# quentinll/pertrenderer

Measured on AMD Instinct MI355X. Metric: rendered frames/sec + ms/backward, 256² img, 50 faces/px, 8 samples, higher is better.
Workload: dtype f32; 1 GPU; cfg2 pose-opt step: sphere_642 (1280 faces), 256x256, faces_per_pixel=50, Sr=Sa=8 Gaussian, sigma=1e-3 gamma=1e-2, blur=ln(1e4-1)*sigma, fwd + L2 loss (native) + bwd + Adam step on the pose (lr 5e-2); image_size=256, faces_per_pixel=50, nb_samples=8, rast_samples=8, batch=1, execution=graph, parallelism=single GPU

## Files before the change

### pertrenderer_amd/csrc/pr_rast.hip

```cpp
#include <cstdlib>
#include <type_traits>

#include <hip/hip_fp16.h>

#include "pr_common.h"

namespace pr {
namespace {

constexpr float kEps = 1e-8f;
constexpr int kTile = 4;

struct V2 {
  float x, y;
};

template <bool FAST = false>
PR_DEV float dv(float a, float b) {
  if constexpr (FAST) return a * __builtin_amdgcn_rcpf(b);
  else return a / b;
}

PR_DEV float edge_fn(V2 p, V2 a, V2 b) { return (p.x - a.x) * (b.y - a.y) - (p.y - a.y) * (b.x - a.x); }

// ... 42 lines not shown

PR_DEV float ndc(int i, int S1, int S2) {
  float range = 2.0f;
  if (S1 > S2) range = ((float)S1 * range) / (float)S2;
  const float off = range / 2.0f;
  return -off + (range * (float)i + off) / (float)S1;
}

struct FaceRec {
  float4 a;
  float4 b;
  float4 c;
  float4 d;
  float4 e;
  float4 f;
};

PR_DEV uint32_t half_bits(__half h) { return (uint32_t)__half_as_ushort(h); }
PR_DEV uint2 pack_box(float xmin, float xmax, float ymin, float ymax) {
  return make_uint2(half_bits(__float2half_rd(xmin)) | (half_bits(__float2half_ru(xmax)) << 16),
                    half_bits(__float2half_rd(ymin)) | (half_bits(__float2half_ru(ymax)) << 16));
}
PR_DEV float4 unpack_box(uint2 b) {
  return make_float4(__half2float(__ushort_as_half((unsigned short)(b.x & 0xffffu))),
                     __half2float(__ushort_as_half((unsigned short)(b.x >> 16))),
                     __half2float(__ushort_as_half((unsigned short)(b.y & 0xffffu))),
                     __half2float(__ushort_as_half((unsigned short)(b.y >> 16))));
}

PR_DEV void write_face_rec(const float v[9], float blur, int cull_backfaces, FaceRec* out, uint2* bbox) {
  const float x0 = v[0], y0 = v[1], z0 = v[2], x1 = v[3], y1 = v[4], z1 = v[5], x2 = v[6], y2 = v[7], z2 = v[8];
  const float r = sqrtf(blur);
  float xmin = fminf(x0, fminf(x1, x2)) - r, xmax = fmaxf(x0, fmaxf(x1, x2)) + r;
  float ymin = fminf(y0, fminf(y1, y2)) - r, ymax = fmaxf(y0, fmaxf(y1, y2)) + r;
  const float zmax = fmaxf(z0, fmaxf(z1, z2));
  const float area = edge_fn(V2{x0, y0}, V2{x1, y1}, V2{x2, y2});
  const bool back = area < 0.f;
  const bool zero_area = area <= kEps && area >= -kEps;
  const bool valid = !(zmax < 0.f || (cull_backfaces && back) || zero_area);
  if (!valid) { xmin = ymin = __builtin_inff(); xmax = ymax = -__builtin_inff(); }
  const float d01x = x1 - x0, d01y = y1 - y0, d12x = x2 - x1, d12y = y2 - y1, d20x = x0 - x2, d20y = y0 - y2;
  FaceRec rec;
  rec.a = make_float4(x0, y0, z0, x1);
  rec.b = make_float4(y1, z1, x2, y2);
  rec.c = make_float4(z2, xmin, xmax, ymin);
  rec.d = make_float4(ymax, edge_fn(V2{x2, y2}, V2{x0, y0}, V2{x1, y1}) + kEps, d01x * d01x + d01y * d01y,
                      d12x * d12x + d12y * d12y);
  rec.e = make_float4(d01x, d01y, d12x, d12y);
  rec.f = make_float4(d20x, d20y, d20x * d20x + d20y * d20y, fminf(z0, fminf(z1, z2)));
  *out = rec;
  *bbox = pack_box(xmin, xmax, ymin, ymax);
}

struct BinGrid {
  int bs, nx, ny, cap;
  int* count;
  int* list;
  int H, W;
};

PR_DEV void bin_rect(const BinGrid& g, int bx, int by, float& xmin, float& xmax, float& ymin, float& ymax) {
  const int c0 = bx * g.bs, c1 = min(c0 + g.bs - 1, g.W - 1), r0 = by * g.bs, r1 = min(r0 + g.bs - 1, g.H - 1);
  xmax = ndc(g.W - 1 - c0, g.W, g.H); xmin = ndc(g.W - 1 - c1, g.W, g.H);
  ymax = ndc(g.H - 1 - r0, g.H, g.W); ymin = ndc(g.H - 1 - r1, g.H, g.W);
}

PR_DEV void pix_range(float vmin, float vmax, int S1, int S2, int& lo, int& hi) {
  float range = 2.0f;
  if (S1 > S2) range = ((float)S1 * range) / (float)S2;
  const float off = range / 2.0f;
  const float ilo = fminf(fmaxf(((vmin + off) * (float)S1 - off) / range, -2.f), (float)S1 + 1.f);
  const float ihi = fminf(fmaxf(((vmax + off) * (float)S1 - off) / range, -2.f), (float)S1 + 1.f);
  lo = max(0, (int)floorf((float)(S1 - 1) - ihi) - 1);
  hi = min(S1 - 1, (int)ceilf((float)(S1 - 1) - ilo) + 1);
}

PR_DEV void bin_face(const BinGrid& g, int n, int64_t f, uint2 packed) {
  const float4 bb = unpack_box(packed);
  if (!(bb.x <= bb.y && bb.z <= bb.w)) return;
  int c0, c1, r0, r1;
  pix_range(bb.x, bb.y, g.W, g.H, c0, c1);
  pix_range(bb.z, bb.w, g.H, g.W, r0, r1);
  if (c0 > c1 || r0 > r1) return;
  const int bx0 = c0 / g.bs, nbx = c1 / g.bs - bx0 + 1, by0 = r0 / g.bs, nby = r1 / g.bs - by0 + 1;
  auto hits = [&](int bx, int by) {
    float xmin, xmax, ymin, ymax;
    bin_rect(g, bx, by, xmin, xmax, ymin, ymax);
    return !(bb.x > xmax || bb.y < xmin || bb.z > ymax || bb.w < ymin);
  };
  if (nbx * nby <= 16) {
    int b[16], c[16];
#pragma unroll
    for (int k = 0; k < 16; ++k) {
      const int bx = bx0 + k % nbx, by = by0 + k / nbx;
      b[k] = k < nbx * nby && hits(bx, by) ? (n * g.ny + by) * g.nx + bx : -1;
    }
#pragma unroll
    for (int k = 0; k < 16; ++k) c[k] = b[k] >= 0 ? atomicAdd(g.count + b[k], 1) : g.cap;
#pragma unroll
    for (int k = 0; k < 16; ++k)
      if (c[k] < g.cap) g.list[(int64_t)b[k] * g.cap + c[k]] = (int)f;
    return;
  }
  for (int by = by0; by < by0 + nby; ++by) {
    for (int bx = bx0; bx < bx0 + nbx; ++bx) {
      if (!hits(bx, by)) continue;
      const int bi = (n * g.ny + by) * g.nx + bx;
      const int c = atomicAdd(g.count + bi, 1);
      if (c < g.cap) g.list[(int64_t)bi * g.cap + c] = (int)f;
    }
  }
}

PR_DEV int mesh_of_sorted(const int64_t* first, int N, int64_t f) {
  int lo = 0, hi = N - 1;
  while (lo < hi) {
    const int mid = (lo + hi + 1) >> 1;
    if (first[mid] <= f) lo = mid;
    else hi = mid - 1;
  }
  return lo;
}

__global__ void face_prep_kernel(const float* fv, int64_t F, float blur_v, const float* blur_dev, int cull_backfaces,
                                 FaceRec* out, uint2* bbox, BinGrid bins, const int64_t* mesh_first, int N) {
  const float blur = blur_dev ? *blur_dev : blur_v;
  for (int64_t f = (int64_t)blockIdx.x * blockDim.x + threadIdx.x; f < F; f += (int64_t)gridDim.x * blockDim.x) {
    float v[9];
#pragma unroll
    for (int i = 0; i < 9; ++i) v[i] = fv[f * 9 + i];
    write_face_rec(v, blur, cull_backfaces, out + f, bbox + f);
    if (bins.count) bin_face(bins, mesh_of_sorted(mesh_first, N, f), f, bbox[f]);
  }
}

PR_DEV int divmod_small(int i, int d, float inv_d, int& r) {
  int q = (int)((float)i * inv_d);
  r = i - q * d;
  if (r < 0) { --q; r += d; }
  else if (r >= d) { ++q; r -= d; }
  return q;
}

PR_DEV bool key_less(float za, int fa, float zb, int fb) { return za < zb || (za == zb && fa < fb); }

PR_DEV float seg_dist2_d(V2 p, V2 a, float bax, float bay, float l2, V2 b) {
  const float bx = p.x - b.x, by = p.y - b.y;
  const float db = bx * bx + by * by;
  float t = (bax * (p.x - a.x) + bay * (p.y - a.y)) / l2;
  t = t < 0.f ? 0.f : (t > 1.f ? 1.f : t);
  const float qx = a.x + t * bax, qy = a.y + t * bay;
  const float dx = p.x - qx, dy = p.y - qy;
  const float ds = dx * dx + dy * dy;
  return l2 <= kEps ? db : ds;
}

template <bool PERSP, bool CLIP>
PR_DEV void face_eval(const FaceRec& r, V2 p, float bc[3], float& pz, bool& inside, float& d) {
  const V2 v0{r.a.x, r.a.y}, v1{r.a.w, r.b.x}, v2{r.b.z, r.b.w};
  const float z0 = r.a.z, z1 = r.b.y, z2 = r.c.x;
  const float area = r.d.y;
  const float e0 = (p.x - v1.x) * r.e.w - (p.y - v1.y) * r.e.z;
  const float e1 = (p.x - v2.x) * r.f.y - (p.y - v2.y) * r.f.x;
  const float e2 = (p.x - v0.x) * r.e.y - (p.y - v0.y) * r.e.x;
  float b[3] = {e0 / area, e1 / area, e2 / area};
  if constexpr (PERSP) {
    const float t0 = b[0] * z1 * z2, t1 = z0 * b[1] * z2, t2 = z0 * z1 * b[2];
    float s = t0 + t1 + t2;
    s = s > kEps ? s : kEps;
    b[0] = t0 / s; b[1] = t1 / s; b[2] = t2 / s;
  }
  if constexpr (CLIP) {
    clip_fwd(b, bc);
  } else {
    bc[0] = b[0]; bc[1] = b[1]; bc[2] = b[2];
  }
  pz = bc[0] * z0 + bc[1] * z1 + bc[2] * z2;
  inside = b[0] > 0.f && b[1] > 0.f && b[2] > 0.f;
  const float d01 = seg_dist2_d(p, v0, r.e.x, r.e.y, r.d.z, v1);
  const float d02 = seg_dist2_d(p, v0, -r.f.x, -r.f.y, r.f.z, v2);
  const float d12 = seg_dist2_d(p, v1, r.e.z, r.e.w, r.d.w, v2);
  d = d01 < d02 ? d01 : d02;
  d = d < d12 ? d : d12;
}

// ... 60 lines not shown
  pz = bc[0] * z0 + bc[1] * z1 + bc[2] * z2;
  const bool inside = b[0] > 0.f && b[1] > 0.f && b[2] > 0.f;
  bool near = dfast < blur - margin;
  if (!inside && !near && !(dfast > blur + margin)) {
    const float d01 = seg_dist2_d(p, v0, r.e.x, r.e.y, r.d.z, v1);
    const float d02 = seg_dist2_d(p, v0, -r.f.x, -r.f.y, r.f.z, v2);
    const float d12 = seg_dist2_d(p, v1, r.e.z, r.e.w, r.d.w, v2);
    float d = d01 < d02 ? d01 : d02;
    d = d < d12 ? d : d12;
    near = d < blur;
  }
  return !(pz < 0.f) && (inside || near);
}

PR_DEV bool in_bbox(const FaceRec& r, V2 p) {
  return !(p.x < r.c.y || p.x > r.c.z || p.y < r.c.w || p.y > r.d.x);
}

#ifdef PR_RAST_PROFILE
constexpr unsigned kProfTiles = 1 << 16;
__device__ long long g_rast_prof[kProfTiles * 16];
#define PR_STAMP(i) (stamp[i] += (long long)__builtin_amdgcn_s_memtime() - t_, t_ = __builtin_amdgcn_s_memtime())
#else
#define PR_STAMP(i) ((void)0)
#endif

template <int SL> struct RastCfg {
  static constexpr int CAP = SL == 1 ? 512 : (SL == 2 ? 256 : 128);
#ifndef PR_RAST_G4
#define PR_RAST_G4 2
#endif
  static constexpr int G = SL == 1 ? 4 : (SL >= 4 ? PR_RAST_G4 : 2);
#ifndef PR_RAST_CH4
#define PR_RAST_CH4 16
#endif
  static constexpr int CH = SL >= 4 ? PR_RAST_CH4 : 64;
  static_assert(CAP <= 8 * 64, "suffix-min pass holds CAP / 64 <= 8 entries per lane");
};
#ifndef PR_RAST_QPAD
template <int SL> constexpr int rast_qpad() { return SL == 4 ? 1 : 0; }
#else
template <int SL> constexpr int rast_qpad() { return PR_RAST_QPAD; }
#endif
#ifndef PR_RAST_MERGE
#define PR_RAST_MERGE 1
#endif
#ifndef PR_RAST_FRAGC
#define PR_RAST_FRAGC 1
#endif
#ifndef PR_RAST_CULLU
#define PR_RAST_CULLU 16
#endif
constexpr int kCullU = PR_RAST_CULLU;

template <int NT>
PR_DEV void bitonic_sort(float* key, int* val, int n2, int tid) {
  for (int k = 2; k <= n2; k <<= 1) {
    for (int j = k >> 1; j > 0; j >>= 1) {
      for (int i = tid; i < n2; i += NT) {
        const int ixj = i ^ j;
        if (ixj > i) {
          const bool up = (i & k) == 0;
          const float a = key[i], b = key[ixj];
          if ((a > b) == up) {
            key[i] = b; key[ixj] = a;
            const int t = val[i]; val[i] = val[ixj]; val[ixj] = t;
          }
        }
      }
      __syncthreads();
    }
  }
}

template <int E>
PR_DEV void wave_bitonic_sort(float (&key)[E], int (&val)[E], int lane) {
#pragma unroll
  for (int k = 2; k <= E * 64; k <<= 1) {
#pragma unroll
    for (int j = k >> 1; j > 0; j >>= 1) {
      if (j >= 64) {
        const int je = j >> 6;
#pragma unroll
        for (int e = 0; e < E; ++e) {
          const int pe = e ^ je;
          if (pe > e) {
            const bool up = ((e * 64 + lane) & k) == 0;
            const float a = key[e], b = key[pe];
            if ((a > b) == up) {
              key[e] = b; key[pe] = a;
              const int t = val[e]; val[e] = val[pe]; val[pe] = t;
            }
          }
        }
      } else {
#pragma unroll
        for (int e = 0; e < E; ++e) {
          const float ok = __shfl_xor(key[e], j);
          const int ov = __shfl_xor(val[e], j);
          const int i = e * 64 + lane;
          const bool up = (i & k) == 0, lower = (lane & j) == 0;
          const bool take = lower == up ? (ok < key[e]) : (ok > key[e]);
          if (take) { key[e] = ok; val[e] = ov; }
        }
      }
    }
// ... 17 lines not shown
PR_HD size_t rast_fwd_wave_bytes(int K) {
  using C = RastCfg<SL>;
  const size_t b = C::CH * sizeof(FaceRec) + (size_t)K * (64 / SL + rast_qpad<SL>()) * 8 + 64 * 4 + C::CH * 12;
  return (b + 15) / 16 * 16;
}

template <int SL>
size_t rast_fwd_lds_sl(int K, int NW) {
  return NW * rast_fwd_wave_bytes<SL>(K) + (size_t)RastCfg<SL>::CAP * 12 + 16;
}

size_t rast_fwd_lds(int K, int SL, int NW = 1) {
  return SL == 8 ? rast_fwd_lds_sl<8>(K, 1)
                 : SL == 4 ? rast_fwd_lds_sl<4>(K, NW) : (SL == 2 ? rast_fwd_lds_sl<2>(K, 1) : rast_fwd_lds_sl<1>(K, 1));
}

template <int SL>
PR_DEV int from_slice(int v, int s) {
  if constexpr (SL == 1) {
    return v;
  } else if constexpr (SL == 2) {
    switch (s) {
      case 0: return __builtin_amdgcn_update_dpp(0, v, 0xA0, 0xf, 0xf, false);
      default: return __builtin_amdgcn_update_dpp(0, v, 0xF5, 0xf, 0xf, false);
    }
  } else if constexpr (SL == 8) {
    return __shfl(v, (int)(__lane_id() & ~7u) | s);
  } else {
    switch (s) {
      case 0: return __builtin_amdgcn_update_dpp(0, v, 0x00, 0xf, 0xf, false);
      case 1: return __builtin_amdgcn_update_dpp(0, v, 0x55, 0xf, 0xf, false);
      case 2: return __builtin_amdgcn_update_dpp(0, v, 0xAA, 0xf, 0xf, false);
      default: return __builtin_amdgcn_update_dpp(0, v, 0xFF, 0xf, 0xf, false);
    }
  }
}

template <int SL>
PR_DEV int quad_rot(int v, int r) {
  if constexpr (SL == 2) {
    return __builtin_amdgcn_update_dpp(0, v, 0xB1, 0xf, 0xf, false);
  } else if constexpr (SL == 8) {
    const unsigned l = __lane_id();
    return __shfl(v, (int)((l & ~7u) | ((l + (unsigned)r) & 7u)));
  } else {
    switch (r) {
      case 1: return __builtin_amdgcn_update_dpp(0, v, 0x39, 0xf, 0xf, false);
      case 2: return __builtin_amdgcn_update_dpp(0, v, 0x4E, 0xf, 0xf, false);
      default: return __builtin_amdgcn_update_dpp(0, v, 0x93, 0xf, 0xf, false);
    }
  }
}

PR_DEV void ring_tile(int b, int m, int& tx, int& ty) {
  int r = (int)(__builtin_sqrtf((float)b) * 0.5f);
  while (4 * (r + 1) * (r + 1) <= b) ++r;
  while (4 * r * r > b) --r;
  const int k = b - 4 * r * r, s = 2 * r + 2, c0 = m / 2 - r - 1;
  if (k < s) { tx = c0 + k; ty = c0; }
  else if (k < 2 * s - 2) { tx = c0 + s - 1; ty = c0 + 1 + (k - s); }
  else if (k < 3 * s - 2) { tx = c0 + s - 1 - (k - (2 * s - 2)); ty = c0 + s - 1; }
  else { tx = c0; ty = c0 + s - 2 - (k - (3 * s - 2)); }
}

#ifndef PR_RAST_WPE
#define PR_RAST_WPE 1
#endif
#ifndef PR_RAST_DUO_WPE
#define PR_RAST_DUO_WPE 1
#endif
template <int SL, bool PERSP, bool CLIP, bool FRAG, int NW>
__global__ void __launch_bounds__(64 * NW, NW == 2 ? PR_RAST_DUO_WPE : PR_RAST_WPE)
    rast_fwd_kernel(PRRastArgs a, const FaceRec* __restrict__ faces, const uint2* __restrict__ fbox, int ring,
                    BinGrid bins) {
  constexpr int TW = SL >= 4 ? 4 : 8, TH = 64 / SL / TW, TP = TW * TH;
  constexpr int kCap = RastCfg<SL>::CAP, kGroup = RastCfg<SL>::G, CH = RastCfg<SL>::CH;
  constexpr int QS = TP + rast_qpad<SL>();
  constexpr int NT = 64 * NW;
  extern __shared__ float smem[];
  const int K = a.K;
  const int tid = threadIdx.x, lane = tid & 63, wv = NW == 2 ? tid >> 6 : 0;
  const int pix = lane / SL, slice = lane % SL;
  const size_t wbytes = rast_fwd_wave_bytes<SL>(K);
  char* wbase = reinterpret_cast<char*>(smem) + wv * wbytes;
  FaceRec* lrec = reinterpret_cast<FaceRec*>(wbase);
  float2* q = reinterpret_cast<float2*>(lrec + CH);
  int* qsz = reinterpret_cast<int*>(q + (size_t)K * QS);
  int* lcf = qsz + 64;
  float* lcs = reinterpret_cast<float*>(lcf + CH);
  float* lmg = lcs + CH;
  int* lfid = reinterpret_cast<int*>(reinterpret_cast<char*>(smem) + NW * wbytes);
  float* lkey = reinterpret_cast<float*>(lfid + kCap);
  float* lsuf = lkey;
  int* lidx = reinterpret_cast<int*>(lkey + kCap);
  int64_t* lctl = reinterpret_cast<int64_t*>(lidx + kCap);
  const int n = blockIdx.z;
  const int H = a.H, W = a.W;
  int tile_x = blockIdx.x, tile_y = blockIdx.y;
  if (ring & 1) {
    const int b = blockIdx.y * gridDim.x + blockIdx.x;
    if (gridDim.y == gridDim.x) {
      ring_tile(b, gridDim.x, tile_x, tile_y);
    } else {
      ring_tile(b >> 1, gridDim.x, tile_x, tile_y);
      tile_y = 2 * tile_y + (b & 1);
    }
  }
  const int row0 = tile_y * TH, col0 = tile_x * TW;
  const int row = row0 + pix / TW, col = col0 + pix % TW;
  const bool inimg = row < H && col < W;
  const V2 p{ndc(W - 1 - min(col, W - 1), W, H), ndc(H - 1 - min(row, H - 1), H, W)};
  const int c1 = min(col0 + TW - 1, W - 1), r1 = min(row0 + TH - 1, H - 1);
  const float txmax = ndc(W - 1 - col0, W, H), txmin = ndc(W - 1 - c1, W, H);
  const float tymax = ndc(H - 1 - row0, H, W), tymin = ndc(H - 1 - r1, H, W);
  const float tcx = 0.5f * (txmin + txmax), tcy = 0.5f * (tymin + tymax);
  const float ptile = fmaxf(fmaxf(fabsf(txmin), fabsf(txmax)), fmaxf(fabsf(tymin), fabsf(tymax)));
  const int64_t fb = a.mesh_first_face[n];
  const int* ids = nullptr;
  int64_t fe = a.mesh_num_faces[n];
  if (bins.count) {
    const int b = (n * bins.ny + row0 / bins.bs) * bins.nx + col0 / bins.bs;
    const int c = bins.count[b];
    if (c <= bins.cap) { ids = bins.list + (int64_t)b * bins.cap; fe = c; }
  }
  constexpr bool clip = CLIP;
  const float blur = a.blur_radius_dev ? *a.blur_radius_dev : a.blur_radius, sqrt_blur = sqrtf(blur);
  int qs = 0;
  float qlast_z = __builtin_inff();
  int qlast_f = 0x7fffffff;
  int64_t base = 0;
#ifdef PR_RAST_PROFILE
  long long stamp[6] = {0, 0, 0, 0, 0, 0}, t_ = __builtin_amdgcn_s_memtime();
  const long long rt0 = __builtin_amdgcn_s_memrealtime();
  int nlist = 0, n_app = 0, n_ins = 0, w_ins = 0;
#endif
  while (base < fe) {
    int nl = 0;
    while (wv == 0 && base < fe && nl <= kCap - 64) {
      uint2 pb[kCullU];
      int fi[kCullU];
#pragma unroll
      for (int u = 0; u < kCullU; ++u) {
        const int64_t i = base + u * 64 + lane;
        const int64_t ic = i < fe ? i : fe - 1;
        fi[u] = ids ? ids[ic] : (int)(fb + ic);
      }
#pragma unroll
      for (int u = 0; u < kCullU; ++u) pb[u] = fbox[fi[u]];
      int64_t next = base + 64 * kCullU;
      bool stop = false;
#pragma unroll
      for (int u = 0; u < kCullU; ++u) {
        const int64_t i = base + u * 64 + lane;
        const float4 bb = unpack_box(pb[u]);
        const bool keep = i < fe && !(bb.x > txmax || bb.y < txmin || bb.z > tymax || bb.w < tymin);
        const uint64_t bal = __ballot(keep);
        const int cnt = __popcll(bal);
        if (!stop && nl + cnt > kCap) { stop = true; next = base + u * 64; }
        if (!stop) {
          if (keep) lfid[nl + __popcll(bal & ((1ull << lane) - 1ull))] = fi[u];
          nl += cnt;
        }
      }
      base = next < fe ? next : fe;
    }
    if constexpr (NW > 1) {
      if (tid == 0) { lctl[0] = base; lctl[1] = nl; }
      __syncthreads();
      base = lctl[0];
      nl = (int)lctl[1];
    }
    __syncthreads();
    PR_STAMP(0);
#ifdef PR_RAST_PROFILE
    nlist += nl;
#endif
    if (nl == 0) continue;
    if (ring & 2) {
      const int t = ring >> 8;
      if (nl >= t + 32) __builtin_amdgcn_s_setprio(3);
      else if (nl >= t + 16) __builtin_amdgcn_s_setprio(2);
      else if (nl >= t) __builtin_amdgcn_s_setprio(1);
    }
    bool done = !inimg;
    int n2 = 64;
    while (n2 < nl) n2 <<= 1;
    for (int i = tid; i < n2; i += NT) {
      float key = __builtin_inff();
      if (i < nl) {
        const FaceRec& r = faces[lfid[i]];
        const float4 ra = r.a, rb = r.b, re = r.e, rf = r.f;
        const float z2 = r.c.x, area = r.d.y;
        const float e0 = (tcx - ra.w) * re.w - (tcy - rb.x) * re.z;
        const float e1 = (tcx - rb.z) * rf.y - (tcy - rb.w) * rf.x;
        const float e2 = (tcx - ra.x) * re.y - (tcy - ra.y) * re.x;
        const float ia = 1.f / area;
        const float zc = (e0 * ia) * ra.z + (e1 * ia) * rb.y + (e2 * ia) * z2;
        const float zmx = fmaxf(ra.z, fmaxf(rb.y, z2));
        key = fminf(fmaxf(zc, rf.w), zmx);
        if (key != key) key = rf.w;
        key = fminf(key, 3.0e38f);
        if (key != key) key = 0.f;
      }
      lkey[i] = key;
      lidx[i] = i < nl ? i : 0x7fffffff;
    }
    __syncthreads();
// ... 365 lines not shown
          }
          tl[u] = t;
          kk[u] = v - e0;
          e[u] = kth(t, kk[u]);
        }
#pragma unroll
        for (int u = 0; u < U; ++u) {
          if (vb + u * NT + tid >= nvalid) break;
          const int fid = __float_as_int(e[u].y);
          const int rr = tl[u] / TW, cc = tl[u] % TW;
          const int64_t o = (((int64_t)n * H + row0 + rr) * W + col0 + cc) * K + kk[u];
          const V2 pp{ndc(W - 1 - (col0 + cc), W, H), ndc(H - 1 - (row0 + rr), H, W)};
          const FaceRec r = faces[fid];
          float bc[3], pz, d;
          bool inside;
          face_eval<PERSP, CLIP>(r, pp, bc, pz, inside, d);
          if (valid_only) {
            a.pix_to_face[o] = (int64_t)fid;
            a.zbuf[o] = e[u].x;
          }
          a.dists[o] = inside ? -d : d;
          a.bary[o * 3 + 0] = bc[0];
          a.bary[o * 3 + 1] = bc[1];
          a.bary[o * 3 + 2] = bc[2];
        }
      }
    }
  }
#ifdef PR_RAST_PROFILE
  __syncthreads();
  PR_STAMP(5);
  int n_app_tot = n_app, n_ins_tot = n_ins;
  for (int o = 32; o > 0; o >>= 1) { n_app_tot += __shfl_xor(n_app_tot, o); n_ins_tot += __shfl_xor(n_ins_tot, o); }
  if (tid == 0) {
    unsigned hw, xcc;
    asm volatile("s_getreg_b32 %0, hwreg(HW_REG_HW_ID)" : "=s"(hw));
    asm volatile("s_getreg_b32 %0, hwreg(HW_REG_XCC_ID)" : "=s"(xcc));
    const unsigned t = (blockIdx.z * gridDim.y + blockIdx.y) * gridDim.x + blockIdx.x;
    if (t < kProfTiles) {
      long long* rec = g_rast_prof + (size_t)t * 16;
      rec[0] = tile_x; rec[1] = tile_y; rec[2] = blockIdx.z; rec[3] = nlist;
      rec[4] = rt0; rec[5] = (long long)__builtin_amdgcn_s_memrealtime();
      rec[6] = (long long)hw | ((long long)(xcc & 0xf) << 32);
      for (int i = 0; i < 6; ++i) rec[7 + i] = stamp[i];
      rec[13] = SL;
      rec[14] = n_app_tot;
      rec[15] = ((long long)n_ins_tot << 32) | (unsigned)w_ins;
    }
  }
#endif
}

template <int SL, bool PERSP, bool CLIP>
void launch_rast_fwd_sl(const PRRastArgs& a, const FaceRec* fr, const uint2* fb, bool frag, size_t lds,
                        const BinGrid& bins, hipStream_t st, int nw) {
  constexpr int TW = SL >= 4 ? 4 : 8, TH = 64 / SL / TW;
  dim3 grid((a.W + TW - 1) / TW, (a.H + TH - 1) / TH, a.N);
  static const bool ring_env = (getenv("PR_RAST_ORDER") ? atoi(getenv("PR_RAST_ORDER")) : 3) & 1;
  static const bool prio_env = getenv("PR_RAST_PRIO") ? atoi(getenv("PR_RAST_PRIO")) != 0 : true;
  static const int prio_t = getenv("PR_RAST_PRIO_T") ? atoi(getenv("PR_RAST_PRIO_T")) & 255 : 40;
  const bool sq = grid.x % 2 == 0 && (grid.y == grid.x || grid.y == 2 * grid.x);
  const int ring = (ring_env && sq ? 1 : 0) | (prio_env ? 2 : 0) | (prio_t << 8);
  ktimer_mark(0, "rast_fwd_kernel", st);
  if constexpr (SL == 4) {
    if (nw == 2) {
      if (frag) rast_fwd_kernel<SL, PERSP, CLIP, true, 2><<<grid, 128, lds, st>>>(a, fr, fb, ring, bins);
      else rast_fwd_kernel<SL, PERSP, CLIP, false, 2><<<grid, 128, lds, st>>>(a, fr, fb, ring, bins);
      ktimer_mark(1, "rast_fwd_kernel", st);
      return;
    }
  }
  if (frag) rast_fwd_kernel<SL, PERSP, CLIP, true, 1><<<grid, 64, lds, st>>>(a, fr, fb, ring, bins);
  else rast_fwd_kernel<SL, PERSP, CLIP, false, 1><<<grid, 64, lds, st>>>(a, fr, fb, ring, bins);
  ktimer_mark(1, "rast_fwd_kernel", st);
}

template <bool PERSP, bool CLIP>
void launch_rast_fwd_pc(const PRRastArgs& a, const FaceRec* fr, const uint2* fb, int sl, bool frag, size_t lds,
                        const BinGrid& bins, hipStream_t st, int nw) {
  if (sl == 8) launch_rast_fwd_sl<8, PERSP, CLIP>(a, fr, fb, frag, lds, bins, st, 1);
  else if (sl == 4) launch_rast_fwd_sl<4, PERSP, CLIP>(a, fr, fb, frag, lds, bins, st, nw);
  else if (sl == 2) launch_rast_fwd_sl<2, PERSP, CLIP>(a, fr, fb, frag, lds, bins, st, 1);
  else launch_rast_fwd_sl<1, PERSP, CLIP>(a, fr, fb, frag, lds, bins, st, 1);
}

void launch_rast_fwd(const PRRastArgs& a, const FaceRec* fr, const uint2* fb, int sl, bool frag, size_t lds,
                     const BinGrid& bins, hipStream_t st, int nw) {
  const bool persp = a.perspective_correct != 0, clip = a.clip_barycentric_coords != 0;
  if (persp && clip) launch_rast_fwd_pc<true, true>(a, fr, fb, sl, frag, lds, bins, st, nw);
  else if (persp) launch_rast_fwd_pc<true, false>(a, fr, fb, sl, frag, lds, bins, st, nw);
  else if (clip) launch_rast_fwd_pc<false, true>(a, fr, fb, sl, frag, lds, bins, st, nw);
  else launch_rast_fwd_pc<false, false>(a, fr, fb, sl, frag, lds, bins, st, nw);
}

template <bool WIDE>
__global__ void __launch_bounds__(kThreads) rast_frag_kernel(PRRastArgs a, int64_t total) {
  using idx_t = typename std::conditional<WIDE, int64_t, uint32_t>::type;
  const bool persp = a.perspective_correct != 0, clip = a.clip_barycentric_coords != 0;
  for (int64_t oo = (int64_t)blockIdx.x * kThreads + threadIdx.x; oo < total; oo += (int64_t)gridDim.x * kThreads) {
    const idx_t o = (idx_t)oo;
    const int64_t fid = a.pix_to_face[o];
    float bc[3] = {-1.f, -1.f, -1.f}, dist = -1.f;
    if (fid >= 0) {
      const idx_t pix = o / (idx_t)a.K;
      const int col = (int)(pix % (idx_t)a.W), row = (int)((pix / (idx_t)a.W) % (idx_t)a.H);
      const V2 pp{ndc(a.W - 1 - col, a.W, a.H), ndc(a.H - 1 - row, a.H, a.W)};
      const float* v = a.face_verts + fid * 9;
      const V2 v0{v[0], v[1]}, v1{v[3], v[4]}, v2{v[6], v[7]};
      float b0[3], b[3];
      bary_fwd(pp, v0, v1, v2, b0);
      if (persp) persp_fwd(b0, v[2], v[5], v[8], b); else { b[0] = b0[0]; b[1] = b0[1]; b[2] = b0[2]; }
      if (clip) clip_fwd(b, bc); else { bc[0] = b[0]; bc[1] = b[1]; bc[2] = b[2]; }
      const bool inside = b[0] > 0.f && b[1] > 0.f && b[2] > 0.f;
      const float d = tri_dist2(pp, v0, v1, v2);
      dist = inside ? -d : d;
    }
    a.dists[o] = dist;
    a.bary[o * 3 + 0] = bc[0];
    a.bary[o * 3 + 1] = bc[1];
    a.bary[o * 3 + 2] = bc[2];
  }
}

PR_DEV void seg_dist2_bwd(V2 p, V2 a, V2 b, float g, V2& ga, V2& gb) {
  const float bax = b.x - a.x, bay = b.y - a.y;
  const float l2 = bax * bax + bay * bay;
  float t;
  if (l2 <= kEps) t = 1.f;
  else {
    t = dv<true>(bax * (p.x - a.x) + bay * (p.y - a.y), l2);
    t = t < 0.f ? 0.f : (t > 1.f ? 1.f : t);
  }
  const float qx = (1.f - t) * a.x + t * b.x, qy = (1.f - t) * a.y + t * b.y;
  const float dx = qx - p.x, dy = qy - p.y;
  ga.x = g * (1.f - t) * 2.f * dx; ga.y = g * (1.f - t) * 2.f * dy;
  gb.x = g * t * 2.f * dx;         gb.y = g * t * 2.f * dy;
}

PR_DEV void tri_dist2_bwd(V2 p, V2 v0, V2 v1, V2 v2, float g, V2 gv[3]) {
  const float e01 = seg_dist2(p, v0, v1), e02 = seg_dist2(p, v0, v2), e12 = seg_dist2(p, v1, v2);
  gv[0] = V2{0.f, 0.f}; gv[1] = V2{0.f, 0.f}; gv[2] = V2{0.f, 0.f};
  if (e01 <= e02 && e01 <= e12) seg_dist2_bwd(p, v0, v1, g, gv[0], gv[1]);
  else if (e02 <= e01 && e02 <= e12) seg_dist2_bwd(p, v0, v2, g, gv[0], gv[2]);
  else seg_dist2_bwd(p, v1, v2, g, gv[1], gv[2]);
}
// ... 380 lines not shown
      continue;
    }
    const float w[3] = {a.bary[s * 3], a.bary[s * 3 + 1], a.bary[s * 3 + 2]};
    const int64_t rows[3] = {attr_row(a, f, 0), attr_row(a, f, 1), attr_row(a, f, 2)};
    float gb[3] = {0.f, 0.f, 0.f};
    for (int d = 0; d < a.D; ++d) {
      const float g = go[d];
#pragma unroll
      for (int i = 0; i < 3; ++i) {
        gb[i] += g * a.face_attr[rows[i] + d];
        if (a.grad_face_attr && g != 0.f) atomicAdd(&a.grad_face_attr[rows[i] + d], w[i] * g);
      }
    }
    if (a.grad_bary) { a.grad_bary[s * 3] = gb[0]; a.grad_bary[s * 3 + 1] = gb[1]; a.grad_bary[s * 3 + 2] = gb[2]; }
  }
}

PR_DEV int mesh_of(const int64_t* first, const int64_t* nf, int N, int64_t f) {
  for (int n = 0; n < N; ++n)
    if (f >= first[n] && f < first[n] + nf[n]) return n;
  return 0;
}

PR_DEV void xform(const float* M, float x, float y, float z, float o[4]) {
#pragma unroll
  for (int c = 0; c < 4; ++c) o[c] = ((x * M[c] + y * M[4 + c]) + z * M[8 + c]) + M[12 + c];
}

__global__ void project_fwd_kernel(PRProjectArgs a) {
  for (int64_t t = (int64_t)blockIdx.x * blockDim.x + threadIdx.x; t < a.F * 3; t += (int64_t)gridDim.x * blockDim.x) {
    const int64_t f = t / 3;
    const int n = mesh_of(a.mesh_first_face, a.mesh_num_faces, a.N, f);
    const float* v = a.verts + a.faces[t] * 3;
    float o[4], c[4];
    xform(a.world_to_view + n * 16, v[0], v[1], v[2], o);
    const float vx = o[0] / o[3], vy = o[1] / o[3], vz = o[2] / o[3];
    xform(a.proj + n * 16, vx, vy, vz, c);
    a.face_verts[t * 3 + 0] = c[0] / c[3];
    a.face_verts[t * 3 + 1] = c[1] / c[3];
    a.face_verts[t * 3 + 2] = vz;
  }
}

__global__ void project_prep_kernel(PRProjectArgs a, float blur_v, const float* blur_dev, int cull_backfaces,
                                    FaceRec* recs, uint2* bbox, float* zero_fv, float* zero_v, BinGrid bins) {
  const int64_t stride = (int64_t)gridDim.x * blockDim.x;
  const float blur = blur_dev ? *blur_dev : blur_v;
  if (a.seed_advance && blockIdx.x == 0 && threadIdx.x == 0) {
    const unsigned i = threadIdx.x;
    uint64_t s = a.seed_advance[i];
    for (int k = 0; k < a.seed_advance_n; ++k) s = seed_next(s);
    a.seed_advance[i] = s;
  }
  for (int64_t f = (int64_t)blockIdx.x * blockDim.x + threadIdx.x; f < a.F; f += stride) {
    const int n = mesh_of(a.mesh_first_face, a.mesh_num_faces, a.N, f);
    float fv[9];
#pragma unroll
    for (int i = 0; i < 3; ++i) {
      const float* v = a.verts + a.faces[f * 3 + i] * 3;
      float o[4], c[4];
      xform(a.world_to_view + n * 16, v[0], v[1], v[2], o);
      const float vx = o[0] / o[3], vy = o[1] / o[3], vz = o[2] / o[3];
      xform(a.proj + n * 16, vx, vy, vz, c);
      fv[i * 3 + 0] = c[0] / c[3];
      fv[i * 3 + 1] = c[1] / c[3];
      fv[i * 3 + 2] = vz;
    }
#pragma unroll
    for (int i = 0; i < 9; ++i) a.face_verts[f * 9 + i] = fv[i];
    write_face_rec(fv, blur, cull_backfaces, recs + f, bbox + f);
    if (bins.count) bin_face(bins, n, f, bbox[f]);
  }
  if (zero_fv)
    for (int64_t i = (int64_t)blockIdx.x * blockDim.x + threadIdx.x; i < a.F * 9; i += stride) zero_fv[i] = 0.f;
  if (zero_v)
    for (int64_t i = (int64_t)blockIdx.x * blockDim.x + threadIdx.x; i < a.V * 3; i += stride) zero_v[i] = 0.f;
}

PR_DEV void project_vertex_bwd(const float* M, const float* P, const float* v, float gx, float gy, float gz,
                               float gout[3]) {
  float o[4], c[4];
  xform(M, v[0], v[1], v[2], o);
  const float vv[3] = {o[0] / o[3], o[1] / o[3], o[2] / o[3]};
  xform(P, vv[0], vv[1], vv[2], c);
  const float i3 = 1.f / c[3], i33 = i3 * i3;
  float gvv[3];
#pragma unroll
  for (int k = 0; k < 3; ++k)
    gvv[k] = gx * (P[k * 4 + 0] * i3 - c[0] * P[k * 4 + 3] * i33) + gy * (P[k * 4 + 1] * i3 - c[1] * P[k * 4 + 3] * i33);
  gvv[2] += gz;
  const float j3 = 1.f / o[3], j33 = j3 * j3;
#pragma unroll
  for (int m = 0; m < 3; ++m) {
    float g = 0.f;
#pragma unroll
    for (int k = 0; k < 3; ++k) g += gvv[k] * (M[m * 4 + k] * j3 - o[k] * M[m * 4 + 3] * j33);
    gout[m] = g;
  }
}

constexpr int kGatherB = 8;
__global__ void project_bwd_gather_kernel(PRProjectArgs a) {
  for (int64_t vi = (int64_t)blockIdx.x * blockDim.x + threadIdx.x; vi < a.V; vi += (int64_t)gridDim.x * blockDim.x) {
    const int64_t s = a.vert_corner_start[vi], e = a.vert_corner_start[vi + 1];
    float g[3] = {0.f, 0.f, 0.f};
    if (s < e) {
      float gx = 0.f, gy = 0.f, gz = 0.f;
      int64_t t0 = 0;
      for (int64_t j0 = s; j0 < e; j0 += kGatherB) {
        int64_t t[kGatherB];
#pragma unroll
        for (int u = 0; u < kGatherB; ++u) t[u] = j0 + u < e ? a.vert_corners[j0 + u] : -1;
        if (j0 == s) t0 = t[0];
        float c[kGatherB][3];
#pragma unroll
        for (int u = 0; u < kGatherB; ++u) {
          if (t[u] >= 0) {
            c[u][0] = a.grad_face_verts[t[u] * 3];
            c[u][1] = a.grad_face_verts[t[u] * 3 + 1];
            c[u][2] = a.grad_face_verts[t[u] * 3 + 2];
          }
        }
#pragma unroll
        for (int u = 0; u < kGatherB; ++u) {
// ... 93 lines not shown
}

extern "C" size_t pr_rast_fwd_workspace_size(const PRRastArgs* a) {
  if (!a) return 0;
  return (size_t)(a->F > 0 ? a->F : 1) * (sizeof(FaceRec) + sizeof(uint2)) + bin_bytes(*a);
}

static int bins_begin(const PRRastArgs& a, BinGrid& g, hipStream_t st) {
  g = bin_grid(a, a.workspace);
  if (!g.count) return PR_OK;
  if (hipMemsetAsync(g.count, 0, (size_t)a.N * g.ny * g.nx * sizeof(int), st) != hipSuccess)
    return set_error(PR_ERR_HIP, "rast_fwd: bin counter memset failed");
  return PR_OK;
}

static int rast_fwd_prepared(const PRRastArgs& a, const FaceRec* fr, const uint2* fbox, const BinGrid& bins,
                             hipStream_t st);

extern "C" int pr_rast_fwd(const PRRastArgs* args, void* stream) {
  if (!args) return set_error(PR_ERR_ARG, "rast_fwd: null args");
  const PRRastArgs& a = *args;
  if (int e = rast_check(a)) return e;
  if (!a.pix_to_face || !a.zbuf || !a.bary || !a.dists) return set_error(PR_ERR_ARG, "rast_fwd: output missing");
  if (!a.workspace || a.workspace_bytes < pr_rast_fwd_workspace_size(args))
    return set_error(PR_ERR_WORKSPACE, "rast_fwd: workspace too small");
  hipStream_t st = reinterpret_cast<hipStream_t>(stream);
  FaceRec* fr = reinterpret_cast<FaceRec*>(a.workspace);
  uint2* fbox = reinterpret_cast<uint2*>(fr + (a.F > 0 ? a.F : 1));
  BinGrid bins;
  if (int e = bins_begin(a, bins, st)) return e;
  if (a.F > 0) {
    const int nb = (int)std::min<int64_t>((a.F + kThreads - 1) / kThreads, 1024);
    face_prep_kernel<<<nb, kThreads, 0, st>>>(a.face_verts, a.F, a.blur_radius, a.blur_radius_dev, a.cull_backfaces, fr,
                                              fbox, bins, a.mesh_first_face, a.N);
    if (int e = check_launch("rast_face_prep")) return e;
  }
  return rast_fwd_prepared(a, fr, fbox, bins, st);
}

static int rast_fwd_prepared(const PRRastArgs& a, const FaceRec* fr, const uint2* fbox, const BinGrid& bins,
                             hipStream_t st) {
  int sl = (int64_t)a.K * 16 * 8 > 16 * 1024 ? 8 : 4;
  if (const char* e = getenv("PR_RAST_SLICES")) {
    const int v = atoi(e);
    if (v == 1 || v == 2 || v == 4 || v == 8) sl = v;
  }
  bool frag = true;
  if (const char* e = getenv("PR_RAST_FRAG")) frag = atoi(e) != 0;
  const char* duo = getenv("PR_RAST_DUO");
  const int nw = sl == 4 && duo && duo[0] == '1' ? 2 : 1;
  size_t lds = rast_fwd_lds(a.K, sl, nw);
  if (const char* e = getenv("PR_RAST_LDS_MIN")) lds = std::max(lds, (size_t)atol(e));
  if (lds > 160 * 1024) return set_error(PR_ERR_ARG, "rast_fwd: faces_per_pixel too large for the LDS queue (max 300)");
  launch_rast_fwd(a, fr, fbox, sl, frag, lds, bins, st, nw);
  if (int e = check_launch("rast_fwd")) return e;
  if (frag) return PR_OK;
  const int64_t total = (int64_t)a.N * a.H * a.W * a.K;
  const int nb = (int)std::min<int64_t>((total + kThreads - 1) / kThreads, 1 << 20);
  if (total * 3 < (int64_t(1) << 32)) rast_frag_kernel<false><<<nb, kThreads, 0, st>>>(a, total);
  else rast_frag_kernel<true><<<nb, kThreads, 0, st>>>(a, total);
  return check_launch("rast_frag");
}

extern "C" size_t pr_rast_bwd_workspace_size(const PRRastArgs* a) {
  if (!a || !(a->flags & PR_DETERMINISTIC)) return 0;
  return detsum_workspace(std::min<int64_t>((int64_t)a->N * a->H * a->W * a->K, det_batch()), a->F, 9);
}

static int rast_bwd_deterministic(const PRRastArgs& a, hipStream_t st) {
  const int64_t total = (int64_t)a.N * a.H * a.W * a.K, batch = det_batch();
  if (a.F == 0) return PR_OK;
  for (int64_t s0 = 0; s0 < total; s0 += batch) {
    const int64_t n = std::min(batch, total - s0);
    DetSum d;
    if (int e = detsum_layout(a.workspace, a.workspace_bytes, n, a.F, 9, d)) return e;
    const int nb = (int)std::min<int64_t>((n + kThreads - 1) / kThreads, 16384);
    rast_bwd_keys_kernel<<<nb, kThreads, 0, st>>>(a, d.keys, s0, n);
    if (int e = check_launch("rast_bwd_keys")) return e;
    if (int e = detsum_sort(d, st)) return e;
    rast_bwd_sorted_grad_kernel<<<nb, kThreads, 0, st>>>(a, d.keys_sorted, d.idx_sorted, d.vals_sorted, s0, n);
    if (int e = check_launch("rast_bwd_sorted_grad")) return e;
    if (int e = detsum_reduce_chain(d, a.grad_face_verts, s0 == 0, st)) return e;
  }
  return PR_OK;
}

extern "C" int pr_rast_bwd(const PRRastArgs* args, void* stream) {
  if (!args) return set_error(PR_ERR_ARG, "rast_bwd: null args");
  const PRRastArgs& a = *args;
  if (int e = rast_check(a)) return e;
  if (!a.pix_to_face || !a.grad_face_verts) return set_error(PR_ERR_ARG, "rast_bwd: buffer missing");
  hipStream_t st = reinterpret_cast<hipStream_t>(stream);
  if (a.flags & PR_DETERMINISTIC) return rast_bwd_deterministic(a, st);
  if (a.F > 0 && !(a.flags & PR_GRAD_PREZEROED)) {
    if (hipMemsetAsync(a.grad_face_verts, 0, (size_t)a.F * 9 * sizeof(float), st) != hipSuccess)
      return set_error(PR_ERR_HIP, "rast_bwd: memset failed");
  }
  const char* er = getenv("PR_RAST_BWD_ROWS");
  const int64_t npix = (int64_t)a.N * a.H * a.W;
  const int rows = er && (atoi(er) == 1 || atoi(er) == 2 || atoi(er) == 4 || atoi(er) == 8) ? atoi(er)
                                                                                            : (npix >= (1 << 18) ? 4 : 2);
  dim3 grid((a.W + kBwdTile - 1) / kBwdTile, (a.H + rows - 1) / rows, a.N);
  static const int order = (getenv("PR_RAST_ORDER") ? atoi(getenv("PR_RAST_ORDER")) : 3) >> 1 & 1;
  static const bool exact = !getenv("PR_RAST_BWD_EXACT") || atoi(getenv("PR_RAST_BWD_EXACT")) != 0;
#define PR_RAST_BWD_LAUNCH(R)                                               \
  do {                                                                      \
    if (exact) rast_bwd_kernel<R, true><<<grid, kBwdThreads, 0, st>>>(a, order);  \
// ... 98 lines not shown
```

Before: 3661 frames/s (fwd+bwd).

## Add hierarchical 64-face chunk bounding boxes to cull chunks in rasterizer

Face prep now reduces the bounding boxes of each 64-face chunk across the wave and stores the union in the bbox slot of the chunk's first face. The exact box of that face stays recoverable from its FaceRec. The forward rasterizer first tests one chunk box per lane against the tile, then checks faces only in surviving chunks, so fewer per-face box reads and tests are needed. This adds a wave reduction in prep, an extra FaceRec read for chunk-leader faces, and more complex control flow. With only 1280 faces (20 chunks), the saving per tile may be small.

```diff
diff --git a/pertrenderer_amd/csrc/pr_rast.hip b/pertrenderer_amd/csrc/pr_rast.hip
--- a/pertrenderer_amd/csrc/pr_rast.hip
+++ b/pertrenderer_amd/csrc/pr_rast.hip
@@ -118,6 +118,28 @@
   *bbox = pack_box(xmin, xmax, ymin, ymax);
 }
 
+constexpr int kChunk = 64;
+
+PR_DEV void write_chunk_box(uint2 packed, bool live, int64_t f, uint2* bbox) {
+  const float inf = __builtin_inff();
+  float4 bb = live ? unpack_box(packed) : make_float4(inf, -inf, inf, -inf);
+  const bool nan = __ballot(bb.x != bb.x || bb.y != bb.y || bb.z != bb.z || bb.w != bb.w) != 0;
+#pragma unroll
+  for (int o = 1; o < kChunk; o <<= 1) {
+    bb.x = fminf(bb.x, __shfl_xor(bb.x, o));
+    bb.y = fmaxf(bb.y, __shfl_xor(bb.y, o));
+    bb.z = fminf(bb.z, __shfl_xor(bb.z, o));
+    bb.w = fmaxf(bb.w, __shfl_xor(bb.w, o));
+  }
+  if (live && (__lane_id() & 63u) == 0)
+    bbox[f] = nan ? pack_box(-inf, inf, -inf, inf) : pack_box(bb.x, bb.y, bb.z, bb.w);
+}
+
+PR_DEV float4 exact_box(const FaceRec* r) {
+  const float4 c = r->c, d = r->d;
+  return make_float4(c.y, c.z, c.w, d.x);
+}
+
 struct BinGrid {
   int bs, nx, ny, cap;
   int* count;
@@ -191,12 +213,20 @@
 __global__ void face_prep_kernel(const float* fv, int64_t F, float blur_v, const float* blur_dev, int cull_backfaces,
                                  FaceRec* out, uint2* bbox, BinGrid bins, const int64_t* mesh_first, int N) {
   const float blur = blur_dev ? *blur_dev : blur_v;
-  for (int64_t f = (int64_t)blockIdx.x * blockDim.x + threadIdx.x; f < F; f += (int64_t)gridDim.x * blockDim.x) {
-    float v[9];
-#pragma unroll
-    for (int i = 0; i < 9; ++i) v[i] = fv[f * 9 + i];
-    write_face_rec(v, blur, cull_backfaces, out + f, bbox + f);
-    if (bins.count) bin_face(bins, mesh_of_sorted(mesh_first, N, f), f, bbox[f]);
+  for (int64_t f0 = (int64_t)blockIdx.x * blockDim.x + (threadIdx.x & ~63u); f0 < F;
+       f0 += (int64_t)gridDim.x * blockDim.x) {
+    const int64_t f = f0 + (threadIdx.x & 63u);
+    const bool live = f < F;
+    uint2 packed = make_uint2(0u, 0u);
+    if (live) {
+      float v[9];
+#pragma unroll
+      for (int i = 0; i < 9; ++i) v[i] = fv[f * 9 + i];
+      write_face_rec(v, blur, cull_backfaces, out + f, bbox + f);
+      packed = bbox[f];
+      if (bins.count) bin_face(bins, mesh_of_sorted(mesh_first, N, f), f, packed);
+    }
+    write_chunk_box(packed, live, f, bbox);
   }
 }
 
@@ -363,6 +393,10 @@
 #define PR_RAST_CULLU 16
 #endif
 constexpr int kCullU = PR_RAST_CULLU;
+#ifndef PR_RAST_CHUNKU
+#define PR_RAST_CHUNKU 16
+#endif
+constexpr int kChunkU = PR_RAST_CHUNKU;
 
 template <int NT>
 PR_DEV void bitonic_sort(float* key, int* val, int n2, int tid) {
@@ -486,6 +520,11 @@
   }
 }
 
+PR_DEV int64_t uniform64(int64_t v) {
+  return (int64_t)(((uint64_t)(uint32_t)__builtin_amdgcn_readfirstlane((int)(v >> 32)) << 32) |
+                   (uint32_t)__builtin_amdgcn_readfirstlane((int)v));
+}
+
 PR_DEV void ring_tile(int b, int m, int& tx, int& ty) {
   int r = (int)(__builtin_sqrtf((float)b) * 0.5f);
   while (4 * (r + 1) * (r + 1) <= b) ++r;
@@ -505,8 +544,8 @@
 #endif
 template <int SL, bool PERSP, bool CLIP, bool FRAG, int NW>
 __global__ void __launch_bounds__(64 * NW, NW == 2 ? PR_RAST_DUO_WPE : PR_RAST_WPE)
-    rast_fwd_kernel(PRRastArgs a, const FaceRec* __restrict__ faces, const uint2* __restrict__ fbox, int ring,
-                    BinGrid bins) {
+    rast_fwd_kernel(PRRastArgs a, const FaceRec* __restrict__ faces, const uint2* __restrict__ fbox,
+                    int chunk_cull, int ring, BinGrid bins) {
   constexpr int TW = SL >= 4 ? 4 : 8, TH = 64 / SL / TW, TP = TW * TH;
   constexpr int kCap = RastCfg<SL>::CAP, kGroup = RastCfg<SL>::G, CH = RastCfg<SL>::CH;
   constexpr int QS = TP + rast_qpad<SL>();
@@ -528,6 +567,7 @@
   float* lsuf = lkey;
   int* lidx = reinterpret_cast<int*>(lkey + kCap);
   int64_t* lctl = reinterpret_cast<int64_t*>(lidx + kCap);
+  int* lscr = reinterpret_cast<int*>(lctl);
   const int n = blockIdx.z;
   const int H = a.H, W = a.W;
   int tile_x = blockIdx.x, tile_y = blockIdx.y;
@@ -570,6 +610,72 @@
 #endif
   while (base < fe) {
     int nl = 0;
+    if (__builtin_amdgcn_readfirstlane(ids == nullptr && wv == 0)) {
+      const int64_t ufb = uniform64(fb), ufe = uniform64(fe);
+      const int f_lo = (int)ufb, f_hi = (int)(ufb + ufe);
+      const int cN = (int)((ufb + ufe - 1) / kChunk) + 1;
+      int64_t ub = uniform64(base);
+      int un = 0;
+      while (ub < ufe && un <= kCap - 64) {
+        const int c0 = (int)((ufb + ub) / kChunk);
+        bool ck = c0 + lane < cN;
+        if (ck && chunk_cull) {
+          const float4 cb = unpack_box(fbox[(c0 + lane) * kChunk]);
+          ck = !(cb.x > txmax || cb.y < txmin || cb.z > tymax || cb.w < tymin);
+        }
+        uint64_t live = __ballot(ck);
+        const int64_t wend = (int64_t)(c0 + 64 < cN ? c0 + 64 : cN) * kChunk - ufb;
+        int64_t next = wend;
+        while (live != 0 && un <= kCap - 64) {
+          uint2 pb[kChunkU];
+          const uint64_t live0 = live;
+          const int nlive = __popcll(live);
+          const int np = nlive < kChunkU ? nlive : kChunkU;
+          int g = -1;
+#pragma unroll
+          for (int u = 0; u < kChunkU; ++u) {
+            pb[u] = make_uint2(0u, 0u);
+            if (u < np) {
+              const int f0 = (c0 + __builtin_ctzll(live)) * kChunk, f = f0 + lane;
+              live &= live - 1;
+              pb[u] = fbox[f >= f_lo && f < f_hi ? f : f_lo];
+              if (lane == u) g = f0;
+            }
+          }
+          float4 ex = make_float4(0.f, 0.f, 0.f, 0.f);
+          if (g >= f_lo && g < f_hi) ex = exact_box(faces + g);
+          uint64_t lv = live0;
+          int stop = -1;
+#pragma unroll
+          for (int u = 0; u < kChunkU; ++u) {
+            if (u < np && stop < 0) {
+              const uint64_t lv0 = lv;
+              const int f = (c0 + __builtin_ctzll(lv)) * kChunk + lane;
+              lv &= lv - 1;
+              float4 bb = unpack_box(pb[u]);
+              const float e0 = __shfl(ex.x, u), e1 = __shfl(ex.y, u), e2 = __shfl(ex.z, u), e3 = __shfl(ex.w, u);
+              if (lane == 0) bb = make_float4(e0, e1, e2, e3);
+              const bool keep = f >= f_lo && f < f_hi && !(bb.x > txmax || bb.y < txmin || bb.z > tymax || bb.w < tymin);
+              const uint64_t bal = __ballot(keep);
+              const int cnt = __popcll(bal);
+              if (un + cnt > kCap) {
+                stop = u;
+                live = lv0;
+              } else {
+                *(keep ? lfid + un + __popcll(bal & ((1ull << lane) - 1ull)) : lscr) = f;
+                un += cnt;
+              }
+            }
+          }
+          next = live != 0 ? (int64_t)(c0 + __builtin_ctzll(live)) * kChunk - ufb : wend;
+          if (stop >= 0) live = 0;
+        }
+        next = next > ub ? next : ub;
+        ub = next < ufe ? next : ufe;
+      }
+      base = ub;
+      nl = un;
+    }
     while (wv == 0 && base < fe && nl <= kCap - 64) {
       uint2 pb[kCullU];
       int fi[kCullU];
@@ -586,7 +692,8 @@
 #pragma unroll
       for (int u = 0; u < kCullU; ++u) {
         const int64_t i = base + u * 64 + lane;
-        const float4 bb = unpack_box(pb[u]);
+        float4 bb = unpack_box(pb[u]);
+        if ((fi[u] & (kChunk - 1)) == 0) bb = exact_box(faces + fi[u]);
         const bool keep = i < fe && !(bb.x > txmax || bb.y < txmin || bb.z > tymax || bb.w < tymin);
         const uint64_t bal = __ballot(keep);
         const int cnt = __popcll(bal);
@@ -1058,7 +1165,7 @@
 }
 
 template <int SL, bool PERSP, bool CLIP>
-void launch_rast_fwd_sl(const PRRastArgs& a, const FaceRec* fr, const uint2* fb, bool frag, size_t lds,
+void launch_rast_fwd_sl(const PRRastArgs& a, const FaceRec* fr, const uint2* fb, int cc, bool frag, size_t lds,
                         const BinGrid& bins, hipStream_t st, int nw) {
   constexpr int TW = SL >= 4 ? 4 : 8, TH = 64 / SL / TW;
   dim3 grid((a.W + TW - 1) / TW, (a.H + TH - 1) / TH, a.N);
@@ -1070,33 +1177,33 @@
   ktimer_mark(0, "rast_fwd_kernel", st);
   if constexpr (SL == 4) {
     if (nw == 2) {
-      if (frag) rast_fwd_kernel<SL, PERSP, CLIP, true, 2><<<grid, 128, lds, st>>>(a, fr, fb, ring, bins);
-      else rast_fwd_kernel<SL, PERSP, CLIP, false, 2><<<grid, 128, lds, st>>>(a, fr, fb, ring, bins);
+      if (frag) rast_fwd_kernel<SL, PERSP, CLIP, true, 2><<<grid, 128, lds, st>>>(a, fr, fb, cc, ring, bins);
+      else rast_fwd_kernel<SL, PERSP, CLIP, false, 2><<<grid, 128, lds, st>>>(a, fr, fb, cc, ring, bins);
       ktimer_mark(1, "rast_fwd_kernel", st);
       return;
     }
   }
-  if (frag) rast_fwd_kernel<SL, PERSP, CLIP, true, 1><<<grid, 64, lds, st>>>(a, fr, fb, ring, bins);
-  else rast_fwd_kernel<SL, PERSP, CLIP, false, 1><<<grid, 64, lds, st>>>(a, fr, fb, ring, bins);
+  if (frag) rast_fwd_kernel<SL, PERSP, CLIP, true, 1><<<grid, 64, lds, st>>>(a, fr, fb, cc, ring, bins);
+  else rast_fwd_kernel<SL, PERSP, CLIP, false, 1><<<grid, 64, lds, st>>>(a, fr, fb, cc, ring, bins);
   ktimer_mark(1, "rast_fwd_kernel", st);
 }
 
 template <bool PERSP, bool CLIP>
-void launch_rast_fwd_pc(const PRRastArgs& a, const FaceRec* fr, const uint2* fb, int sl, bool frag, size_t lds,
-                        const BinGrid& bins, hipStream_t st, int nw) {
-  if (sl == 8) launch_rast_fwd_sl<8, PERSP, CLIP>(a, fr, fb, frag, lds, bins, st, 1);
-  else if (sl == 4) launch_rast_fwd_sl<4, PERSP, CLIP>(a, fr, fb, frag, lds, bins, st, nw);
-  else if (sl == 2) launch_rast_fwd_sl<2, PERSP, CLIP>(a, fr, fb, frag, lds, bins, st, 1);
-  else launch_rast_fwd_sl<1, PERSP, CLIP>(a, fr, fb, frag, lds, bins, st, 1);
-}
-
-void launch_rast_fwd(const PRRastArgs& a, const FaceRec* fr, const uint2* fb, int sl, bool frag, size_t lds,
-                     const BinGrid& bins, hipStream_t st, int nw) {
+void launch_rast_fwd_pc(const PRRastArgs& a, const FaceRec* fr, const uint2* fb, int cc, int sl, bool frag,
+                        size_t lds, const BinGrid& bins, hipStream_t st, int nw) {
+  if (sl == 8) launch_rast_fwd_sl<8, PERSP, CLIP>(a, fr, fb, cc, frag, lds, bins, st, 1);
+  else if (sl == 4) launch_rast_fwd_sl<4, PERSP, CLIP>(a, fr, fb, cc, frag, lds, bins, st, nw);
+  else if (sl == 2) launch_rast_fwd_sl<2, PERSP, CLIP>(a, fr, fb, cc, frag, lds, bins, st, 1);
+  else launch_rast_fwd_sl<1, PERSP, CLIP>(a, fr, fb, cc, frag, lds, bins, st, 1);
+}
+
+void launch_rast_fwd(const PRRastArgs& a, const FaceRec* fr, const uint2* fb, int cc, int sl, bool frag,
+                     size_t lds, const BinGrid& bins, hipStream_t st, int nw) {
   const bool persp = a.perspective_correct != 0, clip = a.clip_barycentric_coords != 0;
-  if (persp && clip) launch_rast_fwd_pc<true, true>(a, fr, fb, sl, frag, lds, bins, st, nw);
-  else if (persp) launch_rast_fwd_pc<true, false>(a, fr, fb, sl, frag, lds, bins, st, nw);
-  else if (clip) launch_rast_fwd_pc<false, true>(a, fr, fb, sl, frag, lds, bins, st, nw);
-  else launch_rast_fwd_pc<false, false>(a, fr, fb, sl, frag, lds, bins, st, nw);
+  if (persp && clip) launch_rast_fwd_pc<true, true>(a, fr, fb, cc, sl, frag, lds, bins, st, nw);
+  else if (persp) launch_rast_fwd_pc<true, false>(a, fr, fb, cc, sl, frag, lds, bins, st, nw);
+  else if (clip) launch_rast_fwd_pc<false, true>(a, fr, fb, cc, sl, frag, lds, bins, st, nw);
+  else launch_rast_fwd_pc<false, false>(a, fr, fb, cc, sl, frag, lds, bins, st, nw);
 }
 
 template <bool WIDE>
@@ -1583,24 +1690,31 @@
     for (int k = 0; k < a.seed_advance_n; ++k) s = seed_next(s);
     a.seed_advance[i] = s;
   }
-  for (int64_t f = (int64_t)blockIdx.x * blockDim.x + threadIdx.x; f < a.F; f += stride) {
-    const int n = mesh_of(a.mesh_first_face, a.mesh_num_faces, a.N, f);
-    float fv[9];
-#pragma unroll
-    for (int i = 0; i < 3; ++i) {
-      const float* v = a.verts + a.faces[f * 3 + i] * 3;
-      float o[4], c[4];
-      xform(a.world_to_view + n * 16, v[0], v[1], v[2], o);
-      const float vx = o[0] / o[3], vy = o[1] / o[3], vz = o[2] / o[3];
-      xform(a.proj + n * 16, vx, vy, vz, c);
-      fv[i * 3 + 0] = c[0] / c[3];
-      fv[i * 3 + 1] = c[1] / c[3];
-      fv[i * 3 + 2] = vz;
-    }
-#pragma unroll
-    for (int i = 0; i < 9; ++i) a.face_verts[f * 9 + i] = fv[i];
-    write_face_rec(fv, blur, cull_backfaces, recs + f, bbox + f);
-    if (bins.count) bin_face(bins, n, f, bbox[f]);
+  for (int64_t f0 = (int64_t)blockIdx.x * blockDim.x + (threadIdx.x & ~63u); f0 < a.F; f0 += stride) {
+    const int64_t f = f0 + (threadIdx.x & 63u);
+    const bool live = f < a.F;
+    uint2 packed = make_uint2(0u, 0u);
+    if (live) {
+      const int n = mesh_of(a.mesh_first_face, a.mesh_num_faces, a.N, f);
+      float fv[9];
+#pragma unroll
+      for (int i = 0; i < 3; ++i) {
+        const float* v = a.verts + a.faces[f * 3 + i] * 3;
+        float o[4], c[4];
+        xform(a.world_to_view + n * 16, v[0], v[1], v[2], o);
+        const float vx = o[0] / o[3], vy = o[1] / o[3], vz = o[2] / o[3];
+        xform(a.proj + n * 16, vx, vy, vz, c);
+        fv[i * 3 + 0] = c[0] / c[3];
+        fv[i * 3 + 1] = c[1] / c[3];
+        fv[i * 3 + 2] = vz;
+      }
+#pragma unroll
+      for (int i = 0; i < 9; ++i) a.face_verts[f * 9 + i] = fv[i];
+      write_face_rec(fv, blur, cull_backfaces, recs + f, bbox + f);
+      packed = bbox[f];
+      if (bins.count) bin_face(bins, n, f, packed);
+    }
+    write_chunk_box(packed, live, f, bbox);
   }
   if (zero_fv)
     for (int64_t i = (int64_t)blockIdx.x * blockDim.x + threadIdx.x; i < a.F * 9; i += stride) zero_fv[i] = 0.f;
@@ -1800,7 +1914,9 @@
   size_t lds = rast_fwd_lds(a.K, sl, nw);
   if (const char* e = getenv("PR_RAST_LDS_MIN")) lds = std::max(lds, (size_t)atol(e));
   if (lds > 160 * 1024) return set_error(PR_ERR_ARG, "rast_fwd: faces_per_pixel too large for the LDS queue (max 300)");
-  launch_rast_fwd(a, fr, fbox, sl, frag, lds, bins, st, nw);
+  const char* cc = getenv("PR_RAST_CHUNK_CULL");
+  const int chunk_cull = !(cc && cc[0] == '0');
+  launch_rast_fwd(a, fr, fbox, chunk_cull, sl, frag, lds, bins, st, nw);
   if (int e = check_launch("rast_fwd")) return e;
   if (frag) return PR_OK;
   const int64_t total = (int64_t)a.N * a.H * a.W * a.K;
```

Result: faster. 3751 frames/s (fwd+bwd) (median of 6 runs) (+2.4%).
